# grunwaldlab/krisp

Measured on AMD Instinct MI355X. Metric: k-mers/s sorted+intersected at k=28, higher is better.
Workload: dtype u64

## Files before the change

include/krisp_hip.h:

```cpp
#ifndef KRISP_HIP_H
#define KRISP_HIP_H

#include <stddef.h>
#include <stdint.h>

#ifdef __cplusplus
extern "C" {
#endif

typedef struct kr_ctx kr_ctx;

typedef struct { uint64_t prefix, in_mask, out_mask; } kr_cand;

typedef struct { uint64_t key; uint32_t genome; uint32_t count; } kr_record;

enum {
    KR_OK = 0,
    KR_ERR_HIP = -1,
    KR_ERR_PARAM = -2,
    KR_ERR_CAPACITY = -3,
    KR_ERR_STATE = -4,
    KR_ERR_KEY = -5,
    KR_ERR_HOST = -6
};
// ... 161 lines not shown
int64_t kr_read_file(const char* path, uint8_t** text, int64_t* stats);
int64_t kr_genome_upload_bgzf(kr_ctx*, int id, const uint8_t* file, size_t n, int one_shot, int64_t* stats);
int64_t kr_genome_upload_gzip(kr_ctx*, int id, const uint8_t* file, size_t n, size_t chunk, int one_shot, int64_t* stats);
int kr_reserve(kr_ctx*, const int* ids, int n, size_t n_bases, int with_text);
int kr_mem_info(kr_ctx*, int64_t* out4);
int64_t kr_genome_upload_text(kr_ctx*, int id, const uint8_t* text, size_t n, int universal_newlines, int one_shot,
                              int64_t* stats);
int64_t kr_genome_fetch_bases(kr_ctx*, int id, uint8_t* out, size_t cap);
void    kr_host_free(void* p);

int64_t kr_scan_special(const uint8_t* bases, size_t n, int k, int omit_soft, uint64_t* starts, size_t cap,
                        int* bad_char);

int64_t kr_render_records(const kr_record* recs, size_t n, int L, int D, int R, const uint32_t* label_of,
                          size_t n_genomes, const char* const* label_text, size_t n_labels, const uint8_t* label_in,
                          int dot, char** csv, size_t* csv_len, char** align, size_t* align_len);
int64_t kr_render_windows(const uint8_t* rows, size_t n, int L, int D, int R, const uint32_t* cand, const uint32_t* genome,
                          const uint32_t* label_of, size_t n_genomes, const char* const* label_text, size_t n_labels,
                          const uint8_t* label_in, int dot, int rna, char** csv, size_t* csv_len, char** align,
                          size_t* align_len);
void    kr_text_free(void* p);

enum { KR_OPT_SLICE_BASES = 1,
       KR_OPT_GENERIC_INTERSECT = 2,
       KR_OPT_ISECT_FORMAT = 3,
       KR_OPT_ABLATE = 4,
       KR_OPT_WIDE_SLOTS = 5,
       KR_OPT_PLACE_TRIES = 7,
       KR_OPT_ISECT_KERNEL = 8,
       KR_OPT_LANES = 9,
       KR_OPT_LAZY_ORDER = 10,
       KR_OPT_COARSE_REST = 11,
       KR_OPT_COARSE_POOL = 12,
       KR_OPT_WIDE_ORDERED = 6 };
int     kr_set_option(kr_ctx*, int option, int64_t value);

int     kr_sync(kr_ctx*);
int     kr_timer_begin(kr_ctx*);
double  kr_timer_end_ms(kr_ctx*);
int     kr_stage_enable(kr_ctx*, int on);
int     kr_stage_select(kr_ctx*, unsigned stage_mask);
int     kr_stage_reset(kr_ctx*);
double  kr_stage_ms(kr_ctx*, int stage);
int64_t kr_stage_launches(kr_ctx*, int stage);

int64_t kr_debug_fetch(kr_ctx*, int genome_id, int what, void* out, size_t cap_bytes);
int64_t kr_debug_inversions(kr_ctx*, int genome_id);
double  kr_debug_localsort(kr_ctx*, int genome_id, int reps, int mode);
double  kr_debug_intersect(kr_ctx*, const int* genome_ids, int n, const uint8_t* is_ingroup, int reps, int mode);
double  kr_debug_copy_gbps(kr_ctx*, size_t bytes, int reps);
const char* kr_debug_copy_which(kr_ctx*);
int     kr_build_experiments(void);
int     kr_debug_lazy(kr_ctx*, int64_t* out8);
int     kr_debug_isect(kr_ctx*, int64_t* out8);
int     kr_debug_scan(kr_ctx*, int64_t* out8);
int     kr_debug_place(kr_ctx*, double* out8);
int     kr_debug_coarse_pool(kr_ctx*, double* out8);
int     kr_debug_comm(kr_ctx*, int64_t* out8);
int     kr_debug_comm_probe(kr_ctx*, size_t bytes, int reps, double* out3);
int64_t kr_debug_cands_selfexchange(kr_ctx*, int apply_filter);
int     kr_debug_comm_hang(kr_ctx*);
int64_t kr_debug_budget_left(kr_ctx*);
int     kr_debug_budget_set(kr_ctx*, int64_t left);
int     kr_debug_info(kr_ctx*, int64_t* out8);

#ifdef __cplusplus
// ... 4 lines not shown
```

krisp_amd/_native.py:

```python
import ctypes
import os

import numpy as np

HERE = os.path.dirname(os.path.abspath(__file__))
LIB_PATH = os.environ.get("KRISP_HIP_LIB") or os.path.join(HERE, "libkrisp_hip.so")

CAND = np.dtype([("prefix", "<u8"), ("in_mask", "<u8"), ("out_mask", "<u8")])
RECORD = np.dtype([("key", "<u8"), ("genome", "<u4"), ("count", "<u4")])
WIDE_HIT = np.dtype([("cand", "<u4"), ("genome", "<u4"), ("pos", "<u4"), ("strand", "<u4")])
LOC_HIT = np.dtype([("group", "<u4"), ("strand", "<u4"), ("pos", "<u8")])
NEAR_HIT = np.dtype([("target", "<u4"), ("strand", "u1"), ("mismatches", "u1"), ("flank_mismatches", "u1"), ("pad", "u1"),
                     ("pos", "<u8")])
PRODUCT_SITE = np.dtype([("pos", "<u8"), ("entry", "<u4"), ("mismatches", "u1"), ("end_mismatches", "u1"),
                         ("pad", "<u2")])
PRODUCT_HIT = np.dtype([("pos", "<u8"), ("length", "<u4"), ("pair", "<u4"), ("strand", "u1"), ("left_mm", "u1"),
                        ("right_mm", "u1"), ("left_end_mm", "u1"), ("right_end_mm", "u1"), ("pad", "u1", (3,))])
DESIGN_RECORD = np.dtype([("found", "<u4"), ("product_size", "<u4"), ("pair_penalty", "<u4"), ("left_start", "<u2"),
                          ("left_len", "<u2"), ("right_start", "<u2"), ("right_len", "<u2"), ("left_tm", "<i4"), ("right_tm", "<i4"),
                          ("left_gc", "<u2"), ("right_gc", "<u2"), ("left_penalty", "<u4"), ("right_penalty", "<u4"),
                          ("left_self_any", "<i4"), ("left_self_end", "<i4"), ("right_self_any", "<i4"),
                          ("right_self_end", "<i4"), ("pair_any", "<i4"), ("pair_end", "<i4")])
DESIGN_RECORD_HP = np.dtype(DESIGN_RECORD.descr + [("left_hairpin", "<i4"), ("right_hairpin", "<i4")])
GUIDE_RECORD = np.dtype([("found", "<u4"), ("strand", "<u4"), ("start", "<u4"), ("min_mismatches", "<u4"),
                         ("sum_mismatches", "<u4"), ("gc", "<u4"), ("candidates", "<u4"), ("pad", "<u4")])
GUIDE_HIT_RAW = np.dtype([("guide", "<u4"), ("strand", "u1"), ("mismatches", "u1"), ("pam", "u1"), ("pad", "u1"), ("pos", "<u8"),
                          ("columns", "<u8")])
GUIDE_BULGE_HIT_RAW = np.dtype([("guide", "<u4"), ("strand", "u1"), ("mismatches", "u1"), ("pam", "u1"), ("bulge", "i1"),
                                ("pos", "<u8"), ("columns", "<u8"), ("bulge_column", "<u4"), ("length", "<u4")])
WIDE_DICT_LEFT, WIDE_DICT_RIGHT, WIDE_GROUPS, WIDE_HITS, WIDE_COUNTS, WIDE_SLOT_BITS, WIDE_NGROUPS, WIDE_BATCH_USED, WIDE_LOCATED, WIDE_KEYS_LISTED = 0, 1, 2, 3, 4, 5, 6, 7, 8, 9
WIDE_MAX_K = 1024
WIDE_MAX_FLANK = 256
COMM_ID_BYTES = 128

SOFT_MAP, SOFT_OMIT = 0, 1
OPT_SLICE_BASES, OPT_GENERIC_INTERSECT, OPT_ISECT_FORMAT, OPT_ABLATE, OPT_WIDE_SLOTS, OPT_WIDE_ORDERED, OPT_PLACE_TRIES = 1, 2, 3, 4, 5, 6, 7
OPT_ISECT_KERNEL = 8
OPT_LANES = 9
OPT_LAZY_ORDER = 10
OPT_COARSE_REST = 11
OPT_COARSE_POOL = 12
ERR_KEY, ERR_HOST = -5, -6
STRANDS_BOTH, STRANDS_FORWARD, STRANDS_CANONICAL = 0, 1, 2
STAGES = ["pack", "hist8", "reduce8", "scatter1", "hist2", "scan2", "scatter2", "chunks", "localsort",
          "fallback", "intersect", "compact", "collect", "merge", "locate"]
STAGE_KERNELS = {"pack": "k_pack", "hist8": "k_hist8 (wide path: k_hist8w, slices: k_hist8k)", "reduce8": "k_reduce8a+k_reduce8b",
                 "scatter1": "k_scatter1p (wide path: k_scatter1w, slices: k_scatter1kp)",
                 "hist2": "k_hist16 (or k_hist2)", "scan2": "k_hist16_off (or k_scan2)", "scatter2": "k_scatter2",
                 "chunks": "k_chunk_table", "localsort": "k_localsort2",
                 "fallback": "k_seg_merge", "intersect": "k_intersect3 (+ k_intersect for oversized items)",
                 "compact": "k_scan+k_publish_reset+k_gather_items",
                 "collect": "k_collect_count+k_tile_sums+k_scan+k_tile_apply+k_publish+k_collect_emit",
                 "merge": "k_cands_flag+k_scan+k_cands_compact", "locate": "k_wide_locate"}

_c = ctypes
_P = _c.c_void_p
SYMBOLS = [
    ("kr_create", _P, [_c.c_int, _c.c_size_t]),
    ("kr_destroy", None, [_P]),
    ("kr_last_error", _c.c_char_p, [_P]),
    ("kr_set_params", _c.c_int, [_P, _c.c_int, _c.c_int, _c.c_int, _c.c_int, _c.c_size_t]),
    ("kr_set_strands", _c.c_int, [_P, _c.c_int]),
    ("kr_genome_upload", _c.c_int, [_P, _c.c_int, _P, _c.c_size_t]),
    ("kr_genome_sort", _c.c_int, [_P, _c.c_int]),
    ("kr_genome_partition", _c.c_int, [_P, _c.c_int]),
    ("kr_genome_add", _c.c_int64, [_P, _c.c_int, _P, _c.c_size_t]),
    ("kr_genome_count", _c.c_int64, [_P, _c.c_int]),
    ("kr_genome_load_sorted", _c.c_int64, [_P, _c.c_int, _P, _c.c_size_t]),
    ("kr_genome_fetch_keys", _c.c_int64, [_P, _c.c_int, _P, _c.c_size_t]),
    ("kr_genome_keys_in_order", _c.c_int64, [_P, _c.c_int, _P, _c.c_size_t]),
    ("kr_set_allow", _c.c_int, [_P, _c.c_uint]),
    ("kr_set_field_order", _c.c_int, [_P, _P, _P]),
    ("kr_set_field_pieces", _c.c_int, [_P, _c.c_int, _P, _P]),
    ("kr_genome_free", _c.c_int, [_P, _c.c_int]),
# ... 737 lines not shown

    def timer_end_ms(self):
        ms = self.lib.kr_timer_end_ms(self.ctx)
        if ms < 0:
            raise KrispHipError("kr_timer_end_ms failed")
        return ms

    def stage_enable(self, on=True):
        self.lib.kr_stage_enable(self.ctx, 1 if on else 0)

    def stage_select(self, names):
        mask = 0
        for n in names:
            mask |= 1 << STAGES.index(n)
        self.lib.kr_stage_select(self.ctx, mask)

    def stage_reset(self):
        self.lib.kr_stage_reset(self.ctx)

    def stage_times(self):
        return {name: (self.lib.kr_stage_ms(self.ctx, i), self.lib.kr_stage_launches(self.ctx, i))
                for i, name in enumerate(STAGES)}

    def debug_info(self):
        o = np.zeros(8, dtype=np.int64)
        self.lib.kr_debug_info(self.ctx, _ptr(o))
        return dict(b=int(o[0]), nbuckets=int(o[1]), T=int(o[2]), CAP=int(o[3]), nwg=int(o[4]),
                    overflow_segments=int(o[5]), fallback_launches=int(o[6]), nslices=int(o[7]))

    def debug_isect(self):
        o = np.zeros(8, dtype=np.int64)
        self.lib.kr_debug_isect(self.ctx, _ptr(o))
        return dict(chunk_kernel_items=int(o[0]), slices_redone=int(o[1]), threads=int(o[2]), buckets_per_item_log2=int(o[3]),
                    heads32=int(o[4]), sort_lanes=int(o[5]))

    def debug_lazy(self):
        o = np.zeros(8, dtype=np.int64)
        self.lib.kr_debug_lazy(self.ctx, _ptr(o))
        return dict(skipped=int(o[0]), ordered_later=int(o[1]), touch_collects=int(o[2]), on=int(o[3]),
                    anchor_in_bucket_order=int(o[4]), fuse_anchor=int(o[5]), coarse=int(o[6]), coarse_promoted=int(o[7]))

    def debug_scan(self):
        o = np.zeros(8, dtype=np.int64)
        self.lib.kr_debug_scan(self.ctx, _ptr(o))
        return dict(tiles=int(o[0]), grid=int(o[1]), cap=int(o[2]), blocks=int(o[3]))

    def copy_gbps(self, nbytes=1 << 30, reps=10):
        v = self.lib.kr_debug_copy_gbps(self.ctx, nbytes, reps)
        if v < 0:
            raise KrispHipError("kr_debug_copy_gbps failed")
        return v

    def mem_info(self):
        o = np.zeros(4, dtype=np.int64)
        self._check(self.lib.kr_mem_info(self.ctx, _ptr(o)), "kr_mem_info")
        return dict(avail=int(o[0]), total=int(o[1]), used=int(o[2]), budget=int(o[3]))

    def debug_comm(self):
        o = np.zeros(8, dtype=np.int64)
        self._check(self.lib.kr_debug_comm(self.ctx, _ptr(o)), "kr_debug_comm")
        return dict(syncs=int(o[0]), p2p=int(o[1]), collectives=int(o[2]), exchange_us=int(o[3]), reduces=int(o[4]),
                    message_entries=int(o[5]))

    def debug_place(self):
        o = np.zeros(8, dtype=np.float64)
        self._check(self.lib.kr_debug_place(self.ctx, _ptr(o)), "kr_debug_place")
        return dict(candidates=int(o[0]), taken=int(o[1]), fastest_ms=[round(float(x), 4) for x in o[2:6]],
# ... 35 lines not shown
```

krisp_amd/csrc/h_core.inc:

```
static thread_local std::string g_last_error;

struct DevBuf {
    void* p = nullptr;
    size_t bytes = 0;
};

struct Slice {
    DevBuf keys, off, chunkstart, chunkdesc, ovf;
    u64 nmax = 0;
    u32 nchunks = 0;
    int64_t count = -1;
    int res = -1;
};

struct Genome {
    int id = -1;
    size_t n_bases = 0;
    u64 nwords = 0;
    u64 nmax = 0;
    DevBuf bases, wkeys;
    DevBuf wlcnt;
    bool wlist = false;
    u32 wlcap = 0;
    std::vector<Slice> sl;
// ... 50 lines not shown
    size_t max_bases = 0;
    std::map<int, Genome> genomes;
    int ls_grid = 768;
    int place_tries = 8;
    bool place_tries_set = false;
    bool shared_gpu = false;
    DevBuf candP;
    DevBuf candA, candB, chunkcnt, chunkpos, flags, blockcnt, blockpos, other, records, nrec, fbdesc, fbsegs;
    DevBuf coltab, collo, colcnt, colpos, coltsum, coltpos, colfirst, colfm;
    int64_t ncand = -1;
    int64_t nrecords = 0;
    std::string err;
    hipEvent_t t0 = nullptr, t1 = nullptr;
    bool stage_on = false;
    unsigned stage_mask = ~0u;
    struct Pair { hipEvent_t a, b; int stage; };
    std::vector<Pair> pending;
    std::vector<hipEvent_t> pool;
    double stage_ms[KR_ST_COUNT] = {0};
    int64_t stage_n[KR_ST_COUNT] = {0};
    int64_t fallback_launches = 0, overflow_segments = 0;
    int dbg = 0;
    int isect_kernel = 0;
    int ncu = 256;
    DevBuf bgz_in, bgz_tab, bgz_stat;
    DevBuf tx_scan;
    DevBuf tx_text, tx_tile, tx_tilepos, tx_lines, tx_ls, tx_ll, tx_op, tx_outpos, tx_state, tx_tsum, tx_tpos;
    u32* mbox = nullptr;
    std::vector<uint64_t> coltab_host;
    std::vector<int> mb_free;
    int mb_next = 0;
    int i3_occ[3][4][9] = {{{0}}};
    DevBuf isovf;
    int64_t isect_ovf_items = 0, isect_refall = 0;
    int i3_last_T = 0, i3_last_mlog = 0, i3_last_tags = 0, i3_last_ua = 0;
    int64_t isect_ua = 0;
    int fuse_anchor = 1;
    u32 i3_ovf_cap = I3_OVF_CAP;
    int isect_fmt = 0;
    int opt_slice_bases = -1;
    hipEvent_t slice_ready[2] = {nullptr, nullptr};
    bool custom_layout = false;
    bool mixed_alphabets = false;
    int lazy_order = 1;
    bool order_wanted = false;
    int64_t lazy_skipped = 0, lazy_ordered = 0, lazy_touch = 0;
    DevBuf touchdesc, touchovf;
    int coarse_rest = 1;
    int64_t coarse_done = 0, coarse_promoted = 0;
    int coarse_pool = 1;
    struct PoolBuf { DevBuf buf; double ms; hipEvent_t ev; bool wait; };
    std::vector<PoolBuf> cpool_free;
    int cpool_total = 0;
    int64_t cpool_partitions = 0;
    int64_t cpool_searches = 0;
    size_t place_min_bytes = (size_t)256 << 20;
    DevBuf co_state, co_tab;
    u32 co_tcap = CO_TCAP;
    u32 co_hitcap = 0;
    int co_occ = 0;
    u32 co_grid = 0;
    u32 scan_cap = 0;
    int64_t scan_dbg[3] = {0, 0, 0};
    int slice_route = 1;
    struct Wide {
        bool on = false;
// ... 342 lines not shown
        g_last_error = "device index out of range";
        return nullptr;
    }
    if (hipSetDevice(device) != hipSuccess) {
        g_last_error = "hipSetDevice failed";
        return nullptr;
    }
    kr_ctx* c = new kr_ctx();
    c->device = device;
    c->budget = hbm_budget_bytes;
    {
        const char* e = getenv("KR_DBG");
        c->dbg = e ? (atoi(e) & 32) : 0;
        const char* e2 = getenv("KR_ISECT_FMT");
        c->isect_fmt = e2 ? (atoi(e2) == 1 ? 1 : (atoi(e2) == 2 ? 2 : 0)) : 0;
        const char* e3 = getenv("KR_SLICE_BASES");
        c->opt_slice_bases = e3 ? std::max(0, std::min(4, atoi(e3))) : -1;
        const char* e16 = getenv("KR_FUSE_ANCHOR");
        c->fuse_anchor = e16 ? atoi(e16) != 0 : 1;
        const char* e15 = getenv("KR_LAZY_ORDER");
        c->lazy_order = e15 ? atoi(e15) != 0 : 1;
        const char* e17 = getenv("KR_COARSE_REST");
        c->coarse_rest = e17 ? atoi(e17) != 0 : 1;
        const char* e21 = getenv("KR_COARSE_POOL");
        c->coarse_pool = e21 ? atoi(e21) != 0 : 1;
        const char* e22 = getenv("KR_PLACE_MIN_BYTES");
        if (e22) c->place_min_bytes = (size_t)std::max(0ll, atoll(e22));
        const char* e18 = getenv("KR_COARSE_TCAP");
        if (e18) c->co_tcap = (u32)std::max(1, std::min((int)CO_TCAP, atoi(e18)));
        const char* e19 = getenv("KR_COARSE_HITCAP");
        if (e19) c->co_hitcap = (u32)std::max(1, atoi(e19));
        const char* e20 = getenv("KR_COARSE_GRID");
        if (e20) c->co_grid = (u32)std::max(0, std::min(65536, atoi(e20)));
        const char* e23 = getenv("KR_SCAN_GRID");
        if (e23) c->scan_cap = (u32)std::max(0, std::min(65536, atoi(e23)));
        const char* e13 = getenv("KR_SLICE_ROUTE");
        c->slice_route = e13 ? atoi(e13) != 0 : 1;
        const char* e8 = getenv("KR_PLACE_TRIES");
        c->place_tries = e8 ? std::max(1, std::min(16, atoi(e8))) : 8;
        c->place_tries_set = e8 != nullptr;
        const char* e4 = getenv("KR_WIDE_SLOTS");
        c->wide.use_slots = e4 ? atoi(e4) != 0 : true;
        const char* e7 = getenv("KR_WIDE_SHARE");
        c->wide.use_share = e7 ? atoi(e7) != 0 : true;
        const char* e11 = getenv("KR_WIDE_SPECTRUM");
        c->wide.packed_spectrum = e11 ? atoi(e11) != 0 : true;
        const char* e5 = getenv("KR_WIDE_ORDERED");
        c->wide.ordered = e5 ? atoi(e5) != 0 : false;
        int ncu = 256, per = 3;
        (void)hipDeviceGetAttribute(&ncu, hipDeviceAttributeMultiprocessorCount, device);
        if (hipOccupancyMaxActiveBlocksPerMultiprocessor(&per, k_localsort2, LS_THREADS, 0) != hipSuccess || per < 1)
            per = 2;
        c->ls_grid = ncu * per;
        c->ncu = ncu;
        const char* e9 = getenv("KR_ISECT_KERNEL");
        c->isect_kernel = e9 ? (atoi(e9) == 1 ? 1 : (atoi(e9) == 2 ? 2 : 0)) : 0;
        const char* e10 = getenv("KR_ISECT_OVF_CAP");
        if (e10) c->i3_ovf_cap = (u32)std::max(0, std::min((int)I3_OVF_CAP, atoi(e10)));
    }
    {
        const char* e = getenv("KR_LANES");
        int nl = e ? atoi(e) : 0;
        c->nlanes = nl < 0 ? 0 : (nl > MAX_LANES ? MAX_LANES : nl);
    }
    bool ok = hipHostMalloc((void**)&c->mbox, MB_WORDS * 4 + PUB_CAP * sizeof(PubEnt), hipHostMallocMapped) == hipSuccess &&
              hipEventCreate(&c->t0) == hipSuccess && hipEventCreate(&c->t1) == hipSuccess &&
// ... 183 lines not shown
    case KR_OPT_WIDE_SLOTS:
        if (value != 0 && value != 1) return fail(c, KR_ERR_PARAM, "KR_OPT_WIDE_SLOTS: 0 or 1");
        c->wide.use_slots = value != 0;
        return KR_OK;
    case KR_OPT_LANES:
        if (value < 0 || value > MAX_LANES) return fail(c, KR_ERR_PARAM, "KR_OPT_LANES: 0 (automatic), 1 .. %d", MAX_LANES);
        HIPCHK(c, hipSetDevice(c->device));
        { int rcj = join_lanes(c); if (rcj) return rcj; }
        HIPCHK(c, hipDeviceSynchronize());
        c->nlanes = (int)value;
        c->next_lane = 0;
        return (c->have_params && c->lane_maxcount) ? ensure_lanes(c, c->lane_maxcount) : KR_OK;
    case KR_OPT_PLACE_TRIES:
        if (value < 1 || value > 16) return fail(c, KR_ERR_PARAM, "KR_OPT_PLACE_TRIES: 1 .. 16");
        c->place_tries = (int)value;
        c->place_tries_set = true;
        return KR_OK;
    case KR_OPT_WIDE_ORDERED:
        if (value != 0 && value != 1) return fail(c, KR_ERR_PARAM, "KR_OPT_WIDE_ORDERED: 0 or 1");
        c->wide.ordered = value != 0;
        return KR_OK;
    case KR_OPT_LAZY_ORDER:
        if (value != 0 && value != 1) return fail(c, KR_ERR_PARAM, "KR_OPT_LAZY_ORDER: 0 or 1");
        c->lazy_order = (int)value;
        return KR_OK;
    case KR_OPT_COARSE_REST:
        if (value != 0 && value != 1) return fail(c, KR_ERR_PARAM, "KR_OPT_COARSE_REST: 0 or 1");
        c->coarse_rest = (int)value;
        return KR_OK;
    case KR_OPT_COARSE_POOL:
        if (value != 0 && value != 1) return fail(c, KR_ERR_PARAM, "KR_OPT_COARSE_POOL: 0 or 1");
        c->coarse_pool = (int)value;
        return KR_OK;
    case KR_OPT_ABLATE:
#ifdef KR_ABLATE
        c->dbg = (c->dbg & 32) | ((int)value & ~32);
        return KR_OK;
#else
        return fail(c, KR_ERR_PARAM, "KR_OPT_ABLATE needs a -DKR_ABLATE build");
#endif
    default:
        return fail(c, KR_ERR_PARAM, "unknown option %d", option);
    }
}

int kr_set_strands(kr_ctx* c, int mode) {
    if (!c || !c->have_params) return fail(c, KR_ERR_STATE, "kr_set_params first");
    if (mode < KR_STRANDS_BOTH || mode > KR_STRANDS_CANONICAL) return fail(c, KR_ERR_PARAM, "unknown strand mode %d", mode);
    if (c->wide.on && mode == KR_STRANDS_CANONICAL) return fail(c, KR_ERR_PARAM, "the wide path emits both strands or the forward one");
    if (!c->genomes.empty()) return fail(c, KR_ERR_STATE, "kr_set_strands after genomes were uploaded");
    c->g.strands = mode;
    c->wide.strands = mode;
    return KR_OK;
}

int kr_set_allow(kr_ctx* c, unsigned base_mask) {
    if (!c || !c->have_params) return fail(c, KR_ERR_STATE, "kr_set_params first");
    if (base_mask > 15) return fail(c, KR_ERR_PARAM, "kr_set_allow: a mask of the four bases A C G T (bits 0..3)");
    if (!c->genomes.empty()) return fail(c, KR_ERR_STATE, "kr_set_allow after genomes were uploaded");
    c->g.allow = base_mask;
    return KR_OK;
}

int kr_set_field_order(kr_ctx* c, const int* widths, const int* order) {
    if (!c || !c->have_params || c->wide.on) return fail(c, KR_ERR_STATE, "kr_set_params first");
    if (!widths || !order) return KR_ERR_PARAM;
// ... 1091 lines not shown
```

krisp_amd/csrc/h_intersect.inc:

```
static int64_t intersect_once(kr_ctx* c, const int* ids, int n, const uint8_t* is_in, int apply_filter, bool* redo);

static int64_t cands_merge_device(kr_ctx* c, size_t m, int have_other, int apply_filter);

static inline int fmode(const kr_ctx* c, int apply_filter) { return apply_filter ? (c->mixed_alphabets ? 2 : 1) : 0; }

int kr_set_mixed_alphabets(kr_ctx* c, int on) {
    if (!c) return KR_ERR_PARAM;
    c->mixed_alphabets = on != 0;
    return KR_OK;
}

#define KR_MAX_CANDS 0xFFFFFF00ull
static int cands_fit(kr_ctx* c, uint64_t n, const char* who) {
    if (n < KR_MAX_CANDS) return KR_OK;
    return fail(c, KR_ERR_CAPACITY, "%s: a candidate list of %llu entries exceeds the %llu a list may hold (an intersection that "
                "nothing prunes: give both ingroup and outgroup genomes to one call, or fewer genomes per call)", who,
                (unsigned long long)n, (unsigned long long)KR_MAX_CANDS);
}

static int cands_compact_room(kr_ctx* c, u32 n) {
    const size_t nblk = ((size_t)n + 255) / 256;
    int rc;
    if ((rc = ensure(c, c->flags, (size_t)n * 4))) return rc;
    if ((rc = ensure(c, c->blockcnt, (nblk + 2) * 4))) return rc;
// ... 238 lines not shown
    if (pending) {
        for (Genome* G : gs)
            if (!G->finalized)
                for (Slice& S : G->sl) open_slices.push_back(&S);
        if (open_slices.size() > PUB_CAP) {
            if ((rc = finalize(c, gs))) return rc;
            pending = false;
        } else {
            if ((rc = join_lanes(c))) return rc;
            publish_slices(c, open_slices.data(), open_slices.size(), c->stream);
        }
    }
    Genome& A = *gs[anchor];
    u64 amax = 0;
    u32 cmax = 0;
    for (Slice& S : A.sl) { amax = std::max(amax, S.nmax); cmax = std::max(cmax, S.nchunks); }
    if ((rc = ensure(c, c->candA, (amax + 2) * sizeof(kr_cand)))) return rc;
    if ((rc = ensure(c, c->candB, 4096 * sizeof(kr_cand)))) return rc;
    if ((rc = ensure(c, c->chunkcnt, ((size_t)cmax + 2) * 4))) return rc;
    if ((rc = ensure(c, c->chunkpos, ((size_t)cmax + 2) * 4))) return rc;
    {
        const size_t nt = ((size_t)std::max(cmax, 1u << c->g.b) + 2047) / 2048 + 8;
        if ((rc = ensure(c, c->coltsum, nt * 4))) return rc;
        if ((rc = ensure(c, c->coltpos, nt * 4))) return rc;
    }
    hipStream_t st = c->stream;
    u64 running = 0;
    const u32 nbk = 1u << c->g.b;
    if (use3) {
        if ((rc = ensure(c, c->chunkcnt, ((size_t)std::max(cmax, nbk) + 2) * 4))) return rc;
        if ((rc = ensure(c, c->chunkpos, ((size_t)std::max(cmax, nbk) + 2) * 4))) return rc;
        if (!c->isovf.p) {
            if ((rc = ensure(c, c->isovf, ((size_t)I3_OVF_CAP + 4) * 4))) return rc;
            HIPCHK(c, hipMemsetAsync(c->isovf.p, 0, 16, st));
        }
    }
    for (int s = 0; s < c->nslices; s++) {
        const Geom g = slice_geom(c, (u32)s);
        Slice& AS = A.sl[s];
        const int fmt = g.D > 8 ? 2 : ((g.D > 4 || c->isect_fmt == 1) ? 1 : 0);
        IsectArgs a{};
        a.n = n;
        a.ingroup_bits = ingroup_bits;
        a.apply_filter = fmode(c, apply_filter);
        a.dbg = c->dbg;
        a.anchor = anchor;
        for (int i = 0; i < n; i++) {
            a.keys[i] = (const u64*)gs[i]->sl[s].keys.p;
            a.off[i] = (const u32*)gs[i]->sl[s].off.p;
        }
        a.chunkdesc = (const uint4*)AS.chunkdesc.p;
        a.tmp = (kr_cand*)c->candA.p;
        a.chunkcnt = (u32*)c->chunkcnt.p;
        auto launch_chunks = [&](u32 grid) {
            hipLaunchKernelGGL(isect_chunk_kernel[fmt], dim3(grid), dim3(IS_THREADS), 0, st, a, g);
        };
        bool by_items = use3;
        u32 nunits = AS.nchunks;
        Isect3Args a3{};
        if (by_items) {
            const ItemPlan ip = item_plan(c, AS, g);
            const int mlog = ip.mlog;
            const u32 T = ip.T;
            const bool tagk = ip.tagk;
            const bool ua = tagk && !gs[anchor]->ordered;
            a3.n = n;
            a3.ingroup_bits = ingroup_bits;
            a3.anchor = anchor;
            a3.apply_filter = a.apply_filter;
            for (int i = 0; i < n; i++) { a3.keys[i] = a.keys[i]; a3.off[i] = a.off[i]; }
            a3.nb = nbk;
            a3.mlog = mlog;
            a3.nitems = (nbk + (1u << mlog) - 1) >> mlog;
            a3.sh = tagk ? ip.sht : std::max(g.rb + mlog - (int)I3_NB_LOG, ip.p0);
            a3.p0 = ip.p0;
            a3.tmp = (kr_cand*)c->candA.p;
            a3.itemcnt = (u32*)c->chunkcnt.p;
            a3.ovf = (u32*)c->isovf.p;
            a3.ovf_cap = c->i3_ovf_cap;
            c->i3_last_T = (int)T;
            c->i3_last_mlog = mlog;
            nunits = a3.nitems;
            c->i3_last_tags = tagk ? 1 : 0;
            const bool st32 = tagk && fmt == 0 && g.D == 1 && n <= 24 && c->isect_fmt == 0;
            const Isect3Kernel kern = isect3_kernel(ua, tagk, st32, fmt);
            int& occ = c->i3_occ[ua ? 2 : (tagk ? 1 : 0)][st32 ? 3 : fmt][T / 64];
            if (occ == 0) {
                int per = 0;
                const hipError_t e = hipOccupancyMaxActiveBlocksPerMultiprocessor(&per, kern, (int)T, 0);
                occ = (e == hipSuccess && per >= 1) ? per : 1;
            }
            const u32 grid = std::min<u32>(a3.nitems, (u32)(occ * c->ncu));
            {
                StageScope sc(c, KR_ST_INTERSECT, st);
                c->i3_last_ua = ua ? 1 : 0;
                if (ua) c->isect_ua++;
                hipLaunchKernelGGL(kern, dim3(grid), dim3(T), 0, st, a3, g);
                a.ovf = (const u32*)c->isovf.p;
                a.ovf_cap = c->i3_ovf_cap;
                a.mlog = mlog;
                a.nb = nbk;
                if (all_ordered) launch_chunks(I3_OVF_LAUNCH);
            }
        } else {
            StageScope sc(c, KR_ST_INTERSECT, st);
            launch_chunks(AS.nchunks);
        }
        u32 total = 0;
        auto gather = [&](u32 cap) {
            if (by_items)
                hipLaunchKernelGGL(k_gather_items, dim3((nunits + GI_ITEMS - 1) / GI_ITEMS), dim3(GI_T), 0, st, g.sbits, g.slice,
                                   (const kr_cand*)c->candA.p, (const u32*)AS.off.p, a3.mlog, nbk,
                                   (const u32*)c->chunkcnt.p, (const u32*)c->chunkpos.p, (kr_cand*)c->candB.p + running,
                                   nunits, cap);
            else
                hipLaunchKernelGGL(k_gather_cands, dim3(AS.nchunks), dim3(64), 0, st, g.sbits, g.slice,
                                   (const kr_cand*)c->candA.p, (const uint4*)AS.chunkdesc.p,
                                   (const u32*)c->chunkcnt.p, (const u32*)c->chunkpos.p,
                                   (kr_cand*)c->candB.p + running, nunits, cap);
        };
        for (;;) {
            u32 novf = 0, cap = 0;
            {
                StageScope sc(c, KR_ST_COMPACT, st);
                if (nunits > 8192) {
                    const u32 nt = (nunits + 2047) / 2048;
                    hipLaunchKernelGGL(k_tile_sums, dim3(nt), dim3(256), 0, st, (const u32*)c->chunkcnt.p, nunits, (u32*)c->coltsum.p);
                    if (nt <= TA2_MAX) {
                        hipLaunchKernelGGL(k_tile_apply2, dim3(nt), dim3(256), 0, st, (const u32*)c->chunkcnt.p, nunits,
                                           (const u32*)c->coltsum.p, nt, (u32*)c->chunkpos.p, c->mbox,
                                           by_items ? (u32*)c->isovf.p : (u32*)nullptr);
                    } else {
                        hipLaunchKernelGGL(k_scan, dim3(1), dim3(1024), 0, st, (const u32*)c->coltsum.p, (u32*)c->coltpos.p, nt);
                        hipLaunchKernelGGL(k_tile_apply, dim3(nt), dim3(256), 0, st, (const u32*)c->chunkcnt.p, nunits,
                                           (const u32*)c->coltpos.p, nt, (u32*)c->chunkpos.p);
                        hipLaunchKernelGGL(k_publish_reset, dim3(1), dim3(64), 0, st, (const u32*)c->chunkpos.p + nunits,
                                           by_items ? (u32*)c->isovf.p : (u32*)nullptr, c->mbox);
                    }
                } else {
                    hipLaunchKernelGGL(k_scan, dim3(1), dim3(1024), 0, st, (const u32*)c->chunkcnt.p, (u32*)c->chunkpos.p, nunits);
                    hipLaunchKernelGGL(k_publish_reset, dim3(1), dim3(64), 0, st, (const u32*)c->chunkpos.p + nunits,
                                       by_items ? (u32*)c->isovf.p : (u32*)nullptr, c->mbox);
                }
                const size_t room = c->candB.bytes / sizeof(kr_cand);
                cap = room > running + 2 ? (u32)std::min<size_t>(room - running - 2, 0xFFFFFFFFu) : 0u;
                gather(cap);
            }
            HIPCHK(c, hipStreamSynchronize(st));
            HIPCHK(c, hipGetLastError());
            total = ((volatile u32*)c->mbox)[0];
            novf = by_items ? ((volatile u32*)c->mbox)[1] : 0u;
            if (by_items && novf > 0 && !all_ordered) {
                if ((rc = ensure_ordered(c, gs))) return rc;
                if ((rc = finalize(c, gs))) return rc;
                *redo = true;
                return 0;
            }
            if (by_items && novf > c->i3_ovf_cap) {
                by_items = false;
                nunits = AS.nchunks;
                a.ovf = nullptr;
                c->isect_refall++;
                StageScope sc2(c, KR_ST_INTERSECT, st);
                launch_chunks(AS.nchunks);
                continue;
            }
            c->isect_ovf_items += novf;
            if (total > cap) {
                StageScope sc(c, KR_ST_COMPACT, st);
                size_t want = running + total + 2;
                if (s == 0 && c->nslices > 1)
                    want = (size_t)((double)total * c->nslices * 1.15) + 4096;
                if ((rc = ensure_keep(c, c->candB, want * sizeof(kr_cand), running * sizeof(kr_cand))))
                    return rc;
                gather(0xFFFFFFFFu);
                HIPCHK(c, hipStreamSynchronize(st));
            }
            break;
        }
        running += total;
        if ((rc = cands_fit(c, running, "kr_intersect"))) return rc;
    }
    HIPCHK(c, hipGetLastError());
    if (pending) {
// ... 316 lines not shown
```

krisp_amd/csrc/h_misc.inc:

```
double kr_debug_localsort(kr_ctx* c, int id, int reps, int mode) {
    if (!c || mode != 0) return -1.0;
    auto it = c->genomes.find(id);
    if (it != c->genomes.end() && ensure_fine(c, it->second)) return -1.0;
    if (it == c->genomes.end() || !it->second.sorted || it->second.sl.empty()) return -1.0;
    if (ensure_ordered(c, {&it->second}) || finalize(c, {&it->second})) return -1.0;
    Slice& S = it->second.sl[0];
    hipStream_t st = c->stream;
    const u32 grid = std::min<u32>(S.nchunks, (u32)c->ls_grid);
    auto launch = [&]() {
        hipLaunchKernelGGL(k_localsort2, dim3(grid), dim3(LS_THREADS), 0, st, (u64*)S.keys.p, (const u32*)S.off.p,
                           (const uint4*)S.chunkdesc.p, S.nchunks, c->g.b, (u32*)S.ovf.p,
                           (uint4*)((char*)S.ovf.p + 16));
    };
    hipEvent_t a, b;
    (void)hipEventCreate(&a);
    (void)hipEventCreate(&b);
    launch();
    (void)hipEventRecord(a, st);
    for (int r = 0; r < reps; r++) launch();
    (void)hipEventRecord(b, st);
    (void)hipEventSynchronize(b);
    float ms = 0;
    (void)hipEventElapsedTime(&ms, a, b);
    (void)hipEventDestroy(a);
// ... 222 lines not shown
    return KR_OK;
}

int kr_debug_coarse_pool(kr_ctx* c, double* out8) {
    if (!c || !out8) return KR_ERR_PARAM;
    int held = 0;
    double lo = 0, hi = 0;
    for (auto& kv : c->genomes) {
        const Genome& G = kv.second;
        if (!G.ckeys.p) continue;
        lo = held ? std::min(lo, G.ckeys_ms) : G.ckeys_ms;
        hi = held ? std::max(hi, G.ckeys_ms) : G.ckeys_ms;
        held++;
    }
    out8[0] = c->cpool_total;
    out8[1] = (double)c->cpool_free.size();
    out8[2] = held;
    out8[3] = (double)c->cpool_partitions;
    out8[4] = (double)c->cpool_searches;
    out8[5] = lo;
    out8[6] = hi;
    out8[7] = c->coarse_pool;
    return KR_OK;
}

int kr_debug_isect(kr_ctx* c, int64_t* o) {
    if (!c || !o) return KR_ERR_PARAM;
    o[0] = c->isect_ovf_items;
    o[1] = c->isect_refall;
    o[2] = c->i3_last_T;
    o[3] = c->i3_last_mlog;
    o[4] = c->i3_last_tags;
    o[5] = lanes_used(c);
    o[6] = o[7] = 0;
    return KR_OK;
}

int kr_debug_scan(kr_ctx* c, int64_t* o) {
    if (!c || !o) return KR_ERR_PARAM;
    o[0] = c->scan_dbg[0];
    o[1] = c->scan_dbg[1];
    o[2] = c->scan_cap;
    o[3] = c->scan_dbg[2];
    o[4] = o[5] = o[6] = o[7] = 0;
    return KR_OK;
}

int kr_build_experiments(void) {
    int bits = 0;
#ifdef KR_EXPERIMENTS
    bits |= 1;
#endif
#ifdef KR_ABLATE
    bits |= 2;
#endif
#if defined(I3_ABL) && I3_ABL
    bits |= 4;
#endif
#if defined(P2_ABL) && P2_ABL
    bits |= 8;
#endif
#ifdef LS2_NORANK
    bits |= 16;
#endif
#ifdef KR_EXP_NOLOOKUP
    bits |= 32;
#endif
// ... 32 lines not shown
```

krisp_amd/csrc/krisp_hip.hip:

```cpp
#include <hip/hip_runtime.h>
#include <rccl/rccl.h>
#include <dlfcn.h>
#include <sys/stat.h>
#include <zlib.h>
#include <unistd.h>

#include <algorithm>
#include <atomic>
#include <chrono>
#include <cstdarg>
#include <cstdio>
#include <cstdlib>
#include <cstring>
#include <cmath>
#include <condition_variable>
#include <cerrno>
#include <map>
#include <memory>
#include <mutex>
#include <string>
#include <thread>
#include <utility>
#include <vector>

#include "krisp_hip.h"

#include "k_keys.inc"
#include "k_sort.inc"
#include "k_sort2.inc"
#include "k_intersect.inc"
#include "k_intersect3.inc"
#include "k_intersect3t.inc"
#include "k_text.inc"
#include "k_inflate.inc"
#include "k_gunzip.inc"
#include "k_wide.inc"
#include "k_scan.inc"
#include "k_locate.inc"
#include "k_near.inc"
#include "k_guide_hits.inc"
#include "k_guide_bulges.inc"

#include "k_products.inc"
#include "k_primers.inc"
#include "k_design.inc"
#include "k_coarse.inc"
#include "k_guides.inc"
#include "h_core.inc"
#include "h_intersect.inc"
#include "h_wide.inc"
#include "h_scan.inc"
#include "h_locate.inc"
#include "h_near.inc"
#include "h_guide_hits.inc"
#include "h_guide_bulges.inc"
#include "h_products.inc"
#include "h_primers.inc"
#include "h_design.inc"
#include "h_guides.inc"
#include "h_pgzip.inc"
#include "h_ingest.inc"
#include "h_gunzip.inc"
#include "h_comm.inc"
#include "h_text.inc"
#include "h_misc.inc"
// ... 3 lines not shown
```

Baseline: 119.6 billion.

## Add hash-screened two-genome join kernel for the intersect stage

```diff
diff --git a/include/krisp_hip.h b/include/krisp_hip.h
--- a/include/krisp_hip.h
+++ b/include/krisp_hip.h
@@ -217,6 +217,7 @@
        KR_OPT_LAZY_ORDER = 10,
        KR_OPT_COARSE_REST = 11,
        KR_OPT_COARSE_POOL = 12,
+       KR_OPT_JOIN2 = 13,
        KR_OPT_WIDE_ORDERED = 6 };
 int     kr_set_option(kr_ctx*, int option, int64_t value);
 
diff --git a/krisp_amd/_native.py b/krisp_amd/_native.py
--- a/krisp_amd/_native.py
+++ b/krisp_amd/_native.py
@@ -40,6 +40,7 @@
 OPT_LAZY_ORDER = 10
 OPT_COARSE_REST = 11
 OPT_COARSE_POOL = 12
+OPT_JOIN2 = 13
 ERR_KEY, ERR_HOST = -5, -6
 STRANDS_BOTH, STRANDS_FORWARD, STRANDS_CANONICAL = 0, 1, 2
 STAGES = ["pack", "hist8", "reduce8", "scatter1", "hist2", "scan2", "scatter2", "chunks", "localsort",
@@ -843,7 +844,7 @@
         o = np.zeros(8, dtype=np.int64)
         self.lib.kr_debug_isect(self.ctx, _ptr(o))
         return dict(chunk_kernel_items=int(o[0]), slices_redone=int(o[1]), threads=int(o[2]), buckets_per_item_log2=int(o[3]),
-                    heads32=int(o[4]), sort_lanes=int(o[5]))
+                    heads32=int(o[4]), sort_lanes=int(o[5]), join2_launches=int(o[6]), join2_handed_on=int(o[7]))
 
     def debug_lazy(self):
         o = np.zeros(8, dtype=np.int64)
diff --git a/krisp_amd/csrc/h_core.inc b/krisp_amd/csrc/h_core.inc
--- a/krisp_amd/csrc/h_core.inc
+++ b/krisp_amd/csrc/h_core.inc
@@ -106,6 +106,11 @@
     int mb_next = 0;
     int i3_occ[3][4][9] = {{{0}}};
     DevBuf isovf;
+    int join2 = 1;
+    u32 j2_grid = 0;
+    int j2_occ[9] = {0};
+    int64_t j2_launches = 0, j2_full = 0;
+    bool j2_full_counted = false;
     int64_t isect_ovf_items = 0, isect_refall = 0;
     int i3_last_T = 0, i3_last_mlog = 0, i3_last_tags = 0, i3_last_ua = 0;
     int64_t isect_ua = 0;
@@ -514,6 +519,10 @@
         if (e19) c->co_hitcap = (u32)std::max(1, atoi(e19));
         const char* e20 = getenv("KR_COARSE_GRID");
         if (e20) c->co_grid = (u32)std::max(0, std::min(65536, atoi(e20)));
+        const char* e24 = getenv("KR_JOIN2");
+        c->join2 = e24 ? atoi(e24) != 0 : 1;
+        const char* e25 = getenv("KR_JOIN2_GRID");
+        if (e25) c->j2_grid = (u32)std::max(0, std::min(65536, atoi(e25)));
         const char* e23 = getenv("KR_SCAN_GRID");
         if (e23) c->scan_cap = (u32)std::max(0, std::min(65536, atoi(e23)));
         const char* e13 = getenv("KR_SLICE_ROUTE");
@@ -763,6 +772,10 @@
         if (value != 0 && value != 1) return fail(c, KR_ERR_PARAM, "KR_OPT_COARSE_POOL: 0 or 1");
         c->coarse_pool = (int)value;
         return KR_OK;
+    case KR_OPT_JOIN2:
+        if (value != 0 && value != 1) return fail(c, KR_ERR_PARAM, "KR_OPT_JOIN2: 0 or 1");
+        c->join2 = (int)value;
+        return KR_OK;
     case KR_OPT_ABLATE:
 #ifdef KR_ABLATE
         c->dbg = (c->dbg & 32) | ((int)value & ~32);
diff --git a/krisp_amd/csrc/h_intersect.inc b/krisp_amd/csrc/h_intersect.inc
--- a/krisp_amd/csrc/h_intersect.inc
+++ b/krisp_amd/csrc/h_intersect.inc
@@ -294,7 +294,7 @@
         if ((rc = ensure(c, c->chunkpos, ((size_t)std::max(cmax, nbk) + 2) * 4))) return rc;
         if (!c->isovf.p) {
             if ((rc = ensure(c, c->isovf, ((size_t)I3_OVF_CAP + 4) * 4))) return rc;
-            HIPCHK(c, hipMemsetAsync(c->isovf.p, 0, 16, st));
+            HIPCHK(c, hipMemsetAsync(c->isovf.p, 0, ((size_t)I3_OVF_CAP + 4) * 4, st));
         }
     }
     for (int s = 0; s < c->nslices; s++) {
@@ -345,18 +345,22 @@
             nunits = a3.nitems;
             c->i3_last_tags = tagk ? 1 : 0;
             const bool st32 = tagk && fmt == 0 && g.D == 1 && n <= 24 && c->isect_fmt == 0;
-            const Isect3Kernel kern = isect3_kernel(ua, tagk, st32, fmt);
-            int& occ = c->i3_occ[ua ? 2 : (tagk ? 1 : 0)][st32 ? 3 : fmt][T / 64];
+            const bool join2 = c->join2 && n == 2 && (ingroup_bits == 1u || ingroup_bits == 2u) && a.apply_filter == 1 &&
+                               g.D == 1 && tagk && ip.p0 >= 2 && c->isect_fmt == 0 && c->isect_kernel == 0 && c->fuse_anchor != 0;
+            const Isect3Kernel kern = join2 ? k_join2 : isect3_kernel(ua, tagk, st32, fmt);
+            int& occ = join2 ? c->j2_occ[T / 64] : c->i3_occ[ua ? 2 : (tagk ? 1 : 0)][st32 ? 3 : fmt][T / 64];
             if (occ == 0) {
                 int per = 0;
                 const hipError_t e = hipOccupancyMaxActiveBlocksPerMultiprocessor(&per, kern, (int)T, 0);
                 occ = (e == hipSuccess && per >= 1) ? per : 1;
             }
-            const u32 grid = std::min<u32>(a3.nitems, (u32)(occ * c->ncu));
+            u32 grid = std::min<u32>(a3.nitems, (u32)(occ * c->ncu));
+            if (join2 && c->j2_grid) grid = std::min(grid, c->j2_grid);
             {
                 StageScope sc(c, KR_ST_INTERSECT, st);
                 c->i3_last_ua = ua ? 1 : 0;
                 if (ua) c->isect_ua++;
+                if (join2) c->j2_launches++;
                 hipLaunchKernelGGL(kern, dim3(grid), dim3(T), 0, st, a3, g);
                 a.ovf = (const u32*)c->isovf.p;
                 a.ovf_cap = c->i3_ovf_cap;
@@ -412,6 +416,13 @@
             HIPCHK(c, hipGetLastError());
             total = ((volatile u32*)c->mbox)[0];
             novf = by_items ? ((volatile u32*)c->mbox)[1] : 0u;
+            if (by_items && novf > 0 && c->j2_launches) {
+                u32 nfull = 0;
+                HIPCHK(c, hipMemcpy(&nfull, (const u32*)c->isovf.p + J2_FULL_WORD, 4, hipMemcpyDeviceToHost));
+                if (nfull) HIPCHK(c, hipMemset((u32*)c->isovf.p + J2_FULL_WORD, 0, 4));
+                if (!c->j2_full_counted) c->j2_full += nfull;
+                c->j2_full_counted = !all_ordered && !c->j2_full_counted;
+            }
             if (by_items && novf > 0 && !all_ordered) {
                 if ((rc = ensure_ordered(c, gs))) return rc;
                 if ((rc = finalize(c, gs))) return rc;
diff --git a/krisp_amd/csrc/h_misc.inc b/krisp_amd/csrc/h_misc.inc
--- a/krisp_amd/csrc/h_misc.inc
+++ b/krisp_amd/csrc/h_misc.inc
@@ -278,7 +278,8 @@
     o[3] = c->i3_last_mlog;
     o[4] = c->i3_last_tags;
     o[5] = lanes_used(c);
-    o[6] = o[7] = 0;
+    o[6] = c->j2_launches;
+    o[7] = c->j2_full;
     return KR_OK;
 }
 
diff --git a/krisp_amd/csrc/j2_screen.inc b/krisp_amd/csrc/j2_screen.inc
--- /dev/null
+++ b/krisp_amd/csrc/j2_screen.inc
@@ -0,0 +1,32 @@
+#include <stdint.h>
+
+#ifndef J2_SCREEN_LOG
+#define J2_SCREEN_LOG 14
+#endif
+#define J2_SCREEN (1u << J2_SCREEN_LOG)
+#ifndef J2_TAB_LOG
+#define J2_TAB_LOG 10
+#endif
+#define J2_TAB (1u << J2_TAB_LOG)
+#ifndef J2_PROBES
+#define J2_PROBES 64u
+#endif
+
+__host__ __device__ inline uint64_t j2_item_key(uint64_t key, int p0, int w) { return (key >> p0) & ((1ull << w) - 1); }
+
+__host__ __device__ inline uint32_t j2_mix(uint64_t ik, uint32_t k0, uint32_t k1) {
+    return (uint32_t)ik * k0 + (uint32_t)(ik >> 32) * k1;
+}
+__host__ __device__ inline uint32_t j2_slot(uint64_t ik) { return j2_mix(ik, 0x9E3779B1u, 0x85EBCA77u) >> (32 - J2_SCREEN_LOG); }
+__host__ __device__ inline uint32_t j2_tab_hash(uint64_t ik) { return j2_mix(ik, 0xC2B2AE3Du, 0x27D4EB2Fu) >> (32 - J2_TAB_LOG); }
+
+__host__ __device__ inline uint32_t j2_bit(uint32_t slot, uint32_t base, bool other) {
+    return 1u << (8u * (slot & 3u) + base + (other ? 4u : 0u));
+}
+__host__ __device__ inline uint32_t j2_byte(uint32_t word, uint32_t slot) { return (word >> (8u * (slot & 3u))) & 255u; }
+
+__host__ __device__ inline bool j2_live(uint32_t a, uint32_t b) {
+    const uint32_t u = (a | b) & 15u;
+    return (a & 15u) != 0 && (b & 15u) != 0 && (u & (u - 1)) != 0;
+}
+__host__ __device__ inline bool j2_live_byte(uint32_t byte) { return j2_live(byte & 15u, byte >> 4); }
diff --git a/krisp_amd/csrc/k_join2.inc b/krisp_amd/csrc/k_join2.inc
--- /dev/null
+++ b/krisp_amd/csrc/k_join2.inc
@@ -0,0 +1,258 @@
+#include "j2_screen.inc"
+
+#ifndef J2_OCC
+#define J2_OCC 6
+#endif
+#define J2_FULL_WORD (I3_OVF_CAP + 2)
+
+__global__ __launch_bounds__(I3_MAXT, J2_OCC) void k_join2(Isect3Args a, Geom g) {
+    __shared__ __attribute__((aligned(16))) u32 scr[J2_SCREEN / 4];
+    __shared__ __attribute__((aligned(16))) unsigned long long tkey[J2_TAB];
+    __shared__ __attribute__((aligned(16))) u32 tst[J2_TAB];
+    __shared__ unsigned long long lkey[J2_TAB];
+    __shared__ u32 lst[J2_TAB];
+    __shared__ uint2 rng[2][MAXG];
+    __shared__ const u64* keyp[MAXG];
+    __shared__ u32 ctl[2];
+    const u32 tid = threadIdx.x, T = blockDim.x, S = 4 * T, G = gridDim.x;
+    const u32 lane = tid & 63;
+    const bool anchor_in = (a.ingroup_bits >> a.anchor) & 1;
+    const int p0 = a.p0, wbits = a.sh + (int)I3T_NB_LOG - a.p0;
+    const u32 prA = 1u << (8 + a.anchor), prB = 1u << (8 + (1 - a.anchor));
+    const u32 sdA = anchor_in ? 1u : 16u, sdB = anchor_in ? 16u : 1u;
+    const u32 og = min(lane >> 1, (u32)a.n - 1);
+    const u32 __attribute__((address_space(1)))* myoff;
+    {
+        u64 mo = (u64)a.off[og];
+        asm volatile("" : "+v"(mo));
+        myoff = (const u32 __attribute__((address_space(1)))*)mo;
+    }
+    auto item_bucket = [&](u32 it, u32 which) {
+        const u64 f = ((u64)it + which) << a.mlog;
+        return (u32)(f < a.nb ? f : a.nb);
+    };
+    for (u32 i = tid; i < J2_SCREEN / 4; i += T) scr[i] = 0;
+    for (u32 i = tid; i < J2_TAB; i += T) { tkey[i] = 0; tst[i] = 0; }
+    if (tid < 2) ctl[tid] = 0;
+    if (tid < (u32)a.n) keyp[tid] = a.keys[tid];
+    {
+        u32 v = myoff[item_bucket(blockIdx.x, lane & 1)];
+        asm volatile("" : "+v"(v));
+        if (tid < 2 * (u32)a.n) {
+            if (lane & 1) rng[0][og].y = v; else rng[0][og].x = v;
+        }
+    }
+    __syncthreads();
+    I3State cur;
+    cur.it = blockIdx.x;
+    cur.g = -1;
+    cur.par = 0;
+    {
+        const uint2 r = rng[0][a.anchor];
+        const u32 s = i3_uni(r.x), e = i3_uni(r.y);
+        cur.over = (e - s > S) ? 1u : 0u;
+        cur.i0 = s;
+        cur.e = cur.over ? s : e;
+    }
+    if (cur.it >= a.nitems) return;
+    u32 item_sa = 0, item_cnt = 0;
+    u32 item_full = 0, item_firstb = 0;
+    u32 voff = 0;
+    I3Regs X, Y, KA;
+    KA.q[0] = KA.q[1] = u32x4{0, 0, 0, 0};
+    i3_issue(X, a, keyp, cur, T);
+
+    auto ikey_of = [&](u32 lo, u32 hi) { return j2_item_key(((u64)hi << 32) | lo, p0, wbits); };
+    auto base_of = [&](u32 lo) { return __builtin_amdgcn_ubfe(lo, (u32)(p0 - 2), 2u); };
+    auto insert = [&](u64 ik, u32 sw) {
+        const unsigned long long want = ik | (1ull << 63);
+        u32 h = j2_tab_hash(ik);
+        bool placed = false;
+        for (u32 t = 0; t < J2_PROBES && !placed; t++) {
+            const unsigned long long old = atomicCAS(&tkey[h], 0ull, want);
+            if (old == 0ull || old == want) {
+                atomicOr(&tst[h], sw);
+                placed = true;
+            }
+            h = (h + 1) & (J2_TAB - 1);
+        }
+        if (!placed) ctl[1] = 1;
+    };
+    auto probe = [&](u64 ik, u32 sw) {
+        const unsigned long long want = ik | (1ull << 63);
+        u32 h = j2_tab_hash(ik);
+        for (u32 t = 0; t < J2_PROBES; t++) {
+            const unsigned long long old = tkey[h];
+            if (old == want) atomicOr(&tst[h], sw);
+            if (old == want || old == 0ull) break;
+            h = (h + 1) & (J2_TAB - 1);
+        }
+    };
+    auto list_item = [&](u32 it, bool full) {
+        const u32 idx = atomicAdd(&a.ovf[0], 1u);
+        if (idx < a.ovf_cap) a.ovf[1 + idx] = it;
+        if (full) atomicAdd(&a.ovf[J2_FULL_WORD], 1u);
+        a.itemcnt[it] = 0;
+    };
+
+    auto advance = [&](I3State& st, u32& pass, u32& b0) {
+        if (st.g >= 0 && st.i0 + S < st.e) {
+            st.i0 += S;
+        } else if (st.g < 0) {
+            const uint2 r = rng[st.par][1 - a.anchor];
+            st.g = 1 - a.anchor;
+            st.i0 = i3_uni(r.x);
+            st.e = st.over ? st.i0 : i3_uni(r.y);
+            b0 = st.i0;
+            pass = 0;
+        } else if (pass == 0 && st.e - b0 > S) {
+            st.i0 = b0;
+            pass = 1;
+        } else {
+            st.it += G;
+            st.par ^= 1u;
+            st.g = -1;
+            pass = 0;
+            const uint2 r = rng[st.par][a.anchor];
+            const u32 s = i3_uni(r.x), e = i3_uni(r.y);
+            st.over = (e - s > S) ? 1u : 0u;
+            st.i0 = s;
+            st.e = st.over ? s : e;
+        }
+        if (st.it >= a.nitems) { st.i0 = 0; st.e = 0; st.over = 0; }
+        st.it = i3_uni(st.it); st.g = (int)i3_uni((u32)st.g); st.i0 = i3_uni(st.i0); st.e = i3_uni(st.e);
+        st.par = i3_uni(st.par); st.over = i3_uni(st.over);
+        pass = i3_uni(pass); b0 = i3_uni(b0);
+    };
+
+    auto process = [&](const I3Regs& R, const I3State& st, const u32 pass, const I3State& nx) {
+        const u32 tid = opaque_tid();
+        asm volatile("" ::"v"(R.q[0]), "v"(R.q[1]));
+        if (st.g < 0) {
+            item_sa = st.i0;
+            item_cnt = st.e - st.i0;
+            item_full = 0;
+            item_firstb = 1;
+            const u32 cnt = item_cnt;
+            if (st.over) {
+                if (tid == 0) list_item(st.it, false);
+            } else {
+#pragma unroll
+                for (int e = 0; e < 4; e++)
+                    if (I3_POS(e) < cnt) {
+                        const u32 slot = j2_slot(ikey_of(I3_LO(R, e), I3_HI(R, e)));
+                        atomicOr(&scr[slot >> 2], j2_bit(slot, base_of(I3_LO(R, e)), false));
+                    }
+                KA = R;
+            }
+            if (tid < 2 * (u32)a.n) {
+                if (lane & 1) rng[st.par ^ 1u][og].y = voff; else rng[st.par ^ 1u][og].x = voff;
+            }
+            __syncthreads();
+        } else if (!st.over) {
+            const u32 cnt = item_cnt;
+            const u32 left = st.e - st.i0;
+            const bool last_of_pass = !(st.i0 + S < st.e);
+            if (item_firstb) {
+                if (tid == 0) ctl[0] = 0;
+                item_firstb = 0;
+            }
+            if (pass == 0) {
+#pragma unroll
+                for (int e = 0; e < 4; e++)
+                    if (I3_POS(e) < left) {
+                        const u32 slot = j2_slot(ikey_of(I3_LO(R, e), I3_HI(R, e)));
+                        atomicOr(&scr[slot >> 2], j2_bit(slot, base_of(I3_LO(R, e)), true));
+                    }
+                if (last_of_pass) {
+                    __syncthreads();
+#pragma unroll
+                    for (int e = 0; e < 4; e++)
+                        if (I3_POS(e) < cnt) {
+                            const u64 ik = ikey_of(I3_LO(KA, e), I3_HI(KA, e));
+                            const u32 slot = j2_slot(ik);
+                            if (j2_live_byte(j2_byte(scr[slot >> 2], slot))) insert(ik, prA | (sdA << base_of(I3_LO(KA, e))));
+                        }
+                    __syncthreads();
+                    item_full = i3_uni(ctl[1]);
+                }
+            }
+            if ((nx.it != st.it || pass == 1) && !item_full) {
+#pragma unroll
+                for (int e = 0; e < 4; e++)
+                    if (I3_POS(e) < left) {
+                        const u64 ik = ikey_of(I3_LO(R, e), I3_HI(R, e));
+                        const u32 slot = j2_slot(ik);
+                        if (j2_live_byte(j2_byte(scr[slot >> 2], slot))) probe(ik, prB | (sdB << base_of(I3_LO(R, e))));
+                    }
+            }
+            if (nx.it != st.it) {
+                __syncthreads();
+                const bool full = item_full != 0;
+                for (u32 i = tid; i < J2_TAB; i += T) {
+                    const unsigned long long k = tkey[i];
+                    if (k != 0ull) {
+                        const u32 s = tst[i];
+                        tkey[i] = 0ull;
+                        tst[i] = 0;
+                        if (!full && (s >> 8) == 3u && (s & (s >> 4) & 15u) == 0) {
+                            const u32 idx = atomicAdd(&ctl[0], 1u);
+                            lkey[idx] = k;
+                            lst[idx] = s;
+                        }
+                    }
+                }
+                for (u32 i = 4 * tid; i < J2_SCREEN / 4; i += 4 * T) *reinterpret_cast<uint4*>(&scr[i]) = make_uint4(0, 0, 0, 0);
+                if (tid == 0) ctl[1] = 0;
+                __syncthreads();
+                const u32 nsurv = full ? 0u : i3_uni(ctl[0]);
+                if (nsurv) {
+                    const u64 base = ((u64)st.it << a.mlog) << g.rb;
+                    const u64 wmask = (1ull << wbits) - 1;
+                    kr_cand* out = a.tmp + item_sa;
+                    for (u32 i = tid; i < nsurv; i += T) {
+                        const unsigned long long k = lkey[i];
+                        const u32 s = lst[i];
+                        u32 r = 0;
+                        for (u32 j = 0; j < nsurv; j++) r += lkey[j] < k ? 1u : 0u;
+                        kr_cand c;
+                        c.prefix = base | ((k & wmask) << p0);
+                        c.in_mask = (u64)(s & 15u);
+                        c.out_mask = (u64)((s >> 4) & 15u);
+                        out[r] = c;
+                    }
+                }
+                if (tid == 0) {
+                    if (full) list_item(st.it, true);
+                    else a.itemcnt[st.it] = nsurv;
+                }
+            }
+        }
+    };
+
+    u32 cur_pass = 0, b0 = 0;
+    for (;;) {
+        I3State nxt = cur;
+        u32 nxt_pass = cur_pass;
+        if (cur.g < 0) {
+            const u32 ni = cur.it + G < a.nitems ? cur.it + G : 0u;
+            voff = myoff[item_bucket(ni, lane & 1)];
+        }
+        advance(nxt, nxt_pass, b0);
+        i3_issue(Y, a, keyp, nxt, T);
+        process(X, cur, cur_pass, nxt);
+        cur = nxt;
+        cur_pass = nxt_pass;
+        if (cur.it >= a.nitems) break;
+        if (cur.g < 0) {
+            const u32 ni = cur.it + G < a.nitems ? cur.it + G : 0u;
+            voff = myoff[item_bucket(ni, lane & 1)];
+        }
+        advance(nxt, nxt_pass, b0);
+        i3_issue(X, a, keyp, nxt, T);
+        process(Y, cur, cur_pass, nxt);
+        cur = nxt;
+        cur_pass = nxt_pass;
+        if (cur.it >= a.nitems) break;
+    }
+}
diff --git a/krisp_amd/csrc/krisp_hip.hip b/krisp_amd/csrc/krisp_hip.hip
--- a/krisp_amd/csrc/krisp_hip.hip
+++ b/krisp_amd/csrc/krisp_hip.hip
@@ -31,6 +31,7 @@
 #include "k_intersect.inc"
 #include "k_intersect3.inc"
 #include "k_intersect3t.inc"
+#include "k_join2.inc"
 #include "k_text.inc"
 #include "k_inflate.inc"
 #include "k_gunzip.inc"
```

After: 123.3 billion (median of 6 runs). 3.1% higher.
